# osmocom/osmo-trx

Measured on AMD Instinct MI355X. Metric: Mbursts/s detect+demod (156.25 sym, 4 SPS), higher is better.
Workload: dtype f32

## Files before the change

### osmo_trx_amd/csrc/trx_kernel_nb.hip

```cpp
#include "trx_k4_common.h"
#include "trx_nb_asm.inc"

#define NB_D_LEN    160
#define NB_CZ_LEN   (TRX_CZ_PAD + TRX_CORR_NARROW + TRX_CZ_PAD)
#define NB_SLICE    (K4_XS + NB_D_LEN + NB_CZ_LEN)
#define NB_COMP_ROWS (TRX_DELAY_FILTS + 1)
#define NB_AMP_FLOATS (8 * 8)
#define NB_TABLES_FLOATS (TRX_SINCV_LDS + 16 * WAVE + NB_COMP_ROWS * 36 + 16 + 8 * 8 + 5 * WAVE + 5 * WAVE + 2 * 8 * 16 + NB_AMP_FLOATS)
#define NB_TABLES_BYTES (NB_TABLES_FLOATS * 4)
#define NB_WPB 16
#define NB_POOL_RING 64
#define NB_POOL_UNSET (-1)
#define NB_POOL_END (-2)
#define NB_NO_BURST 0xffffffffu
#define NB_LDS_TAIL (16 + 4 * NB_POOL_RING)
#define NB_LDS_BYTES (NB_TABLES_BYTES + NB_WPB * NB_SLICE * 8 + NB_LDS_TAIL)
#define NB_MAX_TOA 32



typedef float v3f __attribute__((ext_vector_type(3)));
typedef int v4i __attribute__((ext_vector_type(4)));
typedef int v2i __attribute__((ext_vector_type(2)));
typedef __attribute__((address_space(3))) v2f lds_v2f;

template <typename T>
__device__ __forceinline__ unsigned lds_addr(const T *p)
{
	return (unsigned)(uintptr_t)(const __attribute__((address_space(3))) T *)p;
}

__device__ __forceinline__ int nb_lane_id()
{
	int lane;
	asm volatile("v_mbcnt_lo_u32_b32 %0, -1, 0\n\tv_mbcnt_hi_u32_b32 %0, -1, %0" : "=v"(lane));
	return lane;
}

__global__ void __launch_bounds__(NB_WPB * WAVE)
nb_pull4_kernel(const uint32_t *__restrict__ iq, const trxhip_burst_params *__restrict__ params,
		trxhip_burst_result *__restrict__ results, float *__restrict__ soft, const trx_tables *__restrict__ tab,
		unsigned n_bursts, float thresh, float full_scale, unsigned *__restrict__ pool_ctr, unsigned *__restrict__ redo,
		float gk5, float gk6, float gk7, float gk8)
{
	static_assert(NB_TABLES_BYTES % 16 == 0 && (NB_SLICE * 8) % 16 == 0 && (K4_XS * 8) % 16 == 0 && (NB_D_LEN * 8) % 16 == 0, "16-byte LDS accesses");
	static_assert(NB_LDS_BYTES <= 160 * 1024, "LDS");
	static_assert(NB_ASM_GDEC_OFF == (TRX_SINCV_LDS + 16 * WAVE + NB_COMP_ROWS * 36) * 4, "tools/gen_nb_asm.py: LDS offset of the decimator taps");
	static_assert(NB_ASM_DEC_MAX_NACT == 15 + NB_ASM_CORR_MAX_LEN, "tools/gen_nb_asm.py: DEC and CORR change form at the same window (one test)");
	static_assert(NB_ASM_LSEQ_OFF == (NB_TABLES_FLOATS - NB_AMP_FLOATS - 2 * 8 * 16) * 4, "tools/gen_nb_asm.py: LDS offset of the training-sequence taps");
	static_assert(NB_ASM_AW_PD == (PH_M0 + 52) * 8 && NB_ASM_AW_D == K4_XS * 8 && NB_ASM_AW_CZ == (K4_XS + NB_D_LEN + TRX_CZ_PAD) * 8,
		      "tools/gen_nb_asm.py: offsets of P, D[] and cz[] inside a wave's slice");
	constexpr int NLD = 10;
	extern __shared__ __attribute__((aligned(16))) char smem[];
	const int lane0 = threadIdx.x & (WAVE - 1);
	const int wave = uni((int)(threadIdx.x >> 6));

	float *const sincv = reinterpret_cast<float *>(smem);
	float *const wa4f = sincv + TRX_SINCV_LDS;
	const float4 *const wa4 = reinterpret_cast<const float4 *>(wa4f);
	float *const comp = wa4f + 16 * WAVE;
	float *const gdec = comp + NB_COMP_ROWS * 36;
	float *const lhdr = gdec + 16;
	int *const pkcl = reinterpret_cast<int *>(lhdr + 8 * 8);
	int *const lcn = pkcl + 5 * WAVE;
	c32 *const lseq = reinterpret_cast<c32 *>(lcn + 5 * WAVE);
	float *const lamp = reinterpret_cast<float *>(lseq + 8 * 16);
	c32 *const wbase = reinterpret_cast<c32 *>(smem + NB_TABLES_BYTES) + (size_t)wave * NB_SLICE;
	int *const wg_next = reinterpret_cast<int *>(reinterpret_cast<c32 *>(smem + NB_TABLES_BYTES) + (size_t)NB_WPB * NB_SLICE);
	int *const pool_g = wg_next + 4;
	c32 *const P = wbase;
	c32 *const D = wbase + K4_XS;
	c32 *const cz = D + NB_D_LEN + TRX_CZ_PAD;

	static_assert(4 * TRX_SINCP_STRIDE <= TRX_SINCV_LDS, "the row pairs fit the LUT's LDS space");
	for (int i = threadIdx.x; i < TRX_SINCV_LDS; i += blockDim.x) {
		const int src = trx_sincp_src(i);
		sincv[i] = (src >= 0) ? tab->sincv[src] : 0.0f;
	}
	for (int i = threadIdx.x; i < 16 * WAVE; i += blockDim.x) {
		const int l = i & (WAVE - 1), u = i >> 6;
		const PeakConst pcl = peak_const(l);
		const int q = (u < 8) ? pcl.loA + 512 * (7 - u) : pcl.hiA + 512 * (u - 8);
		wa4f[((u >> 2) * WAVE + l) * 4 + (u & 3)] = (q < TRX_SINCV_LEN) ? tab->sincv[q] : 0.0f;
	}
	for (int i = threadIdx.x; i < NB_COMP_ROWS * 36; i += blockDim.x) {
		const int f = i / 36, j = i % 36;
		comp[i] = (j >= TRX_FUSED_SH) ? tab->comp_filt[f][j - TRX_FUSED_SH] : 0.0f;
	}
	if (threadIdx.x < 16)
		gdec[threadIdx.x] = tab->dec_taps[threadIdx.x];
	if (threadIdx.x < 128)
		lseq[threadIdx.x] = make_float2(tab->seq[TRX_SEQ_TSC0 + (threadIdx.x >> 4)].taps[threadIdx.x & 15].re,
						tab->seq[TRX_SEQ_TSC0 + (threadIdx.x >> 4)].taps[threadIdx.x & 15].im);
	if (threadIdx.x < 64)
		lhdr[threadIdx.x] = reinterpret_cast<const float *>(&tab->seq[TRX_SEQ_TSC0 + (threadIdx.x >> 3)].gain)[threadIdx.x & 7];
	if (threadIdx.x < NB_AMP_FLOATS) {
		const trx_c32 gi = tab->seq[TRX_SEQ_TSC0 + (threadIdx.x >> 3)].gain_inv;
		lamp[threadIdx.x] = trx_amp_lane_coef(gi.re, gi.im, (int)(threadIdx.x & 7));
	}
	if (threadIdx.x < WAVE) {
		const PeakConst pc0 = peak_const(threadIdx.x);
		pkcl[0 * WAVE + threadIdx.x] = pc0.flA;
		pkcl[1 * WAVE + threadIdx.x] = pc0.loA;
		pkcl[2 * WAVE + threadIdx.x] = pc0.hiA;
		pkcl[3 * WAVE + threadIdx.x] = pc0.offB;
		pkcl[4 * WAVE + threadIdx.x] = pc0.ratio_off;
		lcn[2 * threadIdx.x + 0] = pc0.ratio_off * 8;
		lcn[2 * threadIdx.x + 1] = (pc0.flA - 8) * 8;
		lcn[2 * (WAVE + threadIdx.x) + 0] = pc0.offB;
		const int l = threadIdx.x, e = (l - 52) / 3, t = (l - 52) % 3;
		const bool sp = l >= 52;
		lcn[2 * (WAVE + l) + 1] = 8 * (sp ? (t == 0 ? e : t == 1 ? e + 3 : e - 3) : 4 + 3 * (l < 49 ? l : 49));
		lcn[4 * WAVE + l] = sp ? (e + (t == 2 ? 4 : 0)) * K4_NTP * 4 : -1;
	}
	for (int i = lane0; i < NB_SLICE; i += WAVE)
		wbase[i] = make_float2(0.0f, 0.0f);
	if (threadIdx.x == 0) {
		wg_next[0] = NB_WPB;
		wg_next[1] = 0;
	}
	if (threadIdx.x < NB_POOL_RING)
		pool_g[threadIdx.x] = NB_POOL_UNSET;
	__syncthreads();

	const float thr2 = thresh * thresh;
	float gkv = lane0 == 5 ? gk5 : lane0 == 6 ? gk6 : lane0 == 7 ? gk7 : gk8;
	asm volatile("" : "+v"(gkv));
	const float gc0 = thr2 * 1.0001e-5f;
	int t5pk = 0;
	bool t5_ok = true;
	for (int t = 0; t < 8; t++) {
		const int v = (int)(lhdr[8 * t + 5] * 512.0f);
		t5_ok = t5_ok && v >= -8 && v <= 7 && (float)v == lhdr[8 * t + 5] * 512.0f;
		t5pk |= (v & 15) << (4 * t);
	}
	t5pk = uni(t5pk);
	const unsigned toa_lim = (unsigned)uni(t5_ok ? (int)((NB_MAX_TOA + 1u) << 16) : 0);
	const unsigned long long e8_addr = reinterpret_cast<unsigned long long>(&tab->edge8[0][0][0]);
	const unsigned n_wg = gridDim.x;
	const unsigned n_groups = (n_bursts + 15u) >> 4;
	const bool pooled = pool_ctr != nullptr;
	const unsigned n_static_groups = pooled ? ((n_groups - (n_groups >> 3)) / n_wg) * n_wg : n_groups;
	const unsigned n_pool_groups = n_groups - n_static_groups;
	const unsigned gq = n_static_groups / n_wg, gr = n_static_groups % n_wg;
	const unsigned my_groups = gq + (blockIdx.x < gr ? 1u : 0u);
	const unsigned base16 = (blockIdx.x * gq + (blockIdx.x < gr ? blockIdx.x : gr)) << 4;
	unsigned items = my_groups << 4;
	if (base16 + items > n_bursts)
		items = (base16 < n_bursts) ? n_bursts - base16 : 0u;
	auto burst_of = [&](unsigned jj) -> unsigned {
		if (__builtin_expect(jj < items, 1))
			return base16 + jj;
		if (!pooled)
			return NB_NO_BURST;
		const unsigned k = (jj - items) >> 4;
		volatile int *slot = pool_g + (k & (NB_POOL_RING - 1));
		int g;
		while ((g = *slot) == NB_POOL_UNSET)
			__builtin_amdgcn_s_sleep(2);
		g = uni(g);
		if (g < 0)
			return NB_NO_BURST;
// ... 304 lines not shown
				int clip;
				asm("s_cmp_lg_u64 %1, 0\n\ts_cselect_b32 %0, 1, 0" : "=s"(clip) : "s"(__ballot(amax > TRX_CLIP_THRESH)) : "scc");

				const int len = 16 + (int)max_toa;
				__builtin_assume(len >= 16 && len <= 16 + NB_MAX_TOA);
				float v;
				const int lag0 = (len <= NB_ASM_CORR_MAX_LEN) ? NB_ASM_CORR_LANE0 : 0;
				asm volatile(NB_ASM_DECCORR
					     : [nrm] "=&v"(v)
					     : [aw] "v"(a_w), [zero] "v"(0), [len] "s"(len), [tsc] "s"(tsc)
					     : NB_ASM_CLOBBERS);
				{
					DIAG_MARK(3);
					int m_bits, es_bits, bidx;
					v2i kra, kbc;
					int ktp;
					asm volatile(NB_ASM_AMAX("v_lshlrev_b32_e32 v90, 1, %[l4]", "ds_read_b64 %[kra], v90 offset:%c[lc]",
								 "ds_read_b64 %[kbc], v90 offset:%c[lc]+512", "ds_read_b32 %[ktp], %[l4] offset:%c[lc]+1024",
								 "s_nop 0", "s_nop 0", "s_nop 0", "s_nop 0")
						     "s_sub_u32 %[bidx], %[bidx], %[lag0]\n\t"
						     "s_waitcnt lgkmcnt(0)"
						     : [m] "=&s"(m_bits), [es] "=&s"(es_bits), [bidx] "=&s"(bidx), [kra] "=&v"(kra), [kbc] "=&v"(kbc), [ktp] "=&v"(ktp)
						     : [nrm] "v"(v), [ep] "v"(epart), [l4] "v"(a_l4), [lag0] "s"(lag0),
						       [lc] "n"((TRX_SINCV_LDS + 16 * WAVE + NB_COMP_ROWS * 36 + 16 + 64 + 5 * WAVE) * 4)
						     : NB_ASM_CLOBBERS);
					DIAG_MARK(4);
					int st, e512;
					float km;
					asm volatile(NB_ASM_DETA
						     : [st] "=&" NB_ASM_ST(st), [e] "=&s"(e512), [km] "=&v"(km)
						     : [bidx] "s"(bidx), [len] "s"(len), [czb] "s"(lds_addr(cz)), [m] "s"(m_bits), [kr] "v"(kra.x), [ka] "v"(kra.y), [l16] "v"(a_l16),
						       [gkv] "v"(gkv), [c0] "v"(gc0)
						     : NB_ASM_CLOBBERS_ST);
					DIAG_MARK(5);
					int toa512 = 0, xr_bits = 0, xi_bits = 0;
					if (__builtin_expect(st == 1, 1)) {
						asm volatile(NB_ASM_DETB
							     : [st] "=&" NB_ASM_ST(st), [toa] "=&s"(toa512), [xr] "=&s"(xr_bits), [xi] "=&s"(xi_bits)
							     : [e] "s"(e512), [kb] "v"(kbc.x), [czb] "s"(lds_addr(cz)), [km] "v"(km)
							     : NB_ASM_CLOBBERS_ST);
						DIAG_MARK(6);
					}
					if (__builtin_expect(st != 1, 0)) {
						int stc = st;
						asm volatile("" : "+s"(stc));
						if (stc == 3) {
							const int lane = nb_lane_id();
							if (lane == 0)
								atomicAdd(&g_trx_fast_stats[0], 1ull);
							PeakConst pkc;
							pkc.flA = pkcl[0 * WAVE + lane]; pkc.loA = pkcl[1 * WAVE + lane]; pkc.hiA = pkcl[2 * WAVE + lane];
							pkc.offB = pkcl[3 * WAVE + lane]; pkc.ratio_off = pkcl[4 * WAVE + lane];
							c32 xcorr;
							peak_detect_spec<true>(cz, bidx, sincv, pkc, lane, &toa512, &xcorr, wa4);
							toa512 = uni(toa512);
							xr_bits = uni(__float_as_int(xcorr.x));
							xi_bits = uni(__float_as_int(xcorr.y));
							st = 1;
						} else if (stc == 2) {
							if (nb_lane_id() == 0) atomicAdd(&g_trx_fast_stats[2], 1ull);
							mark_left(b);
							keep = 0;
						} else {
							const float energy = __int_as_float(es_bits) * 0.0125f;
							const float rssi = rssi_db(full_scale, energy);
							const uint32_t flags = ((uint32_t)clip << 8) | (1u << 16);
							int word = clip ? -TRXHIP_SIGERR_CLIP : 0;
							word = put_lane<1>(word, 0.0f);
							word = put_lane<2>(word, 0.0f);
							word = put_lane<3>(word, 0.0f);
							word = put_lane<4>(word, 0.0f);
							word = put_lane<5>(word, energy);
							word = put_lane<6>(word, rssi);
							word = write_lane<7>(word, (int)flags);
							recw = word;
							o = (v3f){ 0.0f, 0.0f, 0.0f };
							pend_rm = 0xff;
						}
					}
					if (__builtin_expect(st == 1, 1)) {
						int ok, s_bits;
						float d0, d1, d2;
						const int t5 = (t5pk << (28 - 4 * tsc)) >> 28;
						asm volatile("s_setprio 0");
						asm volatile(NB_ASM_TAIL
							     : [ok] "=&s"(ok), [ssum] "=&s"(s_bits), [d0] "=&v"(d0), [d1] "=&v"(d1), [d2] "=&v"(d2)
							     : [toa] "s"(toa512), [xr] "s"(xr_bits), [xi] "s"(xi_bits), [t5] "s"(t5), [ampb] "s"(lds_addr(lamp) + 32u * (unsigned)tsc),
							       [e8lo] "s"((unsigned)e8_addr), [e8hi] "s"((unsigned)(e8_addr >> 32)), [l16] "v"(a_l16), [l4] "v"(a_l4),
							       [aw] "v"(a_w), [pb] "s"(lds_addr(P)), [cb] "s"(lds_addr(comp) + 4u * (K4_U0 + TRX_FUSED_SH)), [db] "s"(lds_addr(D)),
							       [kic] "v"(kbc.y), [ktp] "v"(ktp)
							     : NB_ASM_CLOBBERS);
						DIAG_MARK(10);
						asm volatile("s_setprio 2");
						o.x = d0;
						o.y = d1;
						o.z = d2;
						queue_record(xr_bits, xi_bits, es_bits, toa512 - t5 - 10 * 512, s_bits,
							     (int)((uint32_t)tsc | ((uint32_t)clip << 8) | (37u << 24)), b);
						if (__builtin_expect(!ok, 0)) {
							const int lane = nb_lane_id();
							if (lane == 0) atomicAdd(&g_trx_fast_stats[3], 1ull);
							const float *const h = lhdr + 8 * tsc;
							const float xr = __int_as_float(xr_bits), xi = __int_as_float(xi_bits);
							const float a0 = xr * h[2], a1 = xr * h[3], a2 = xi * h[3], a3 = xi * h[2];
							const c32 ampv = make_float2(unif(a0 - a2), unif(a1 + a3));
							if (!demod_general(t5 + 10 * 512 - toa512, ampv, lane)) {
								q_n--;
// ... 32 lines not shown
```

### osmo_trx_amd/csrc/trx_nb_asm.inc

```
#define NB_ASM_GDEC_OFF 29968
#define NB_ASM_LSEQ_OFF 32848
#define NB_ASM_DEC_MAX_NACT 60
#define NB_ASM_CORR_LANE0 19
#define NB_ASM_CORR_MAX_LEN 45
#define NB_ASM_AW_PD 512
#define NB_ASM_AW_D 5760
#define NB_ASM_AW_CZ 7136
#define NB_ASM_ST "{s98}"
#define NB_ASM_CLOBBERS "v64", "v65", "v66", "v67", "v68", "v69", "v70", "v71", "v72", "v73", "v74", "v75", "v76", "v77", "v78", "v79", "v80", "v81", "v82", "v83", "v84", "v85", "v86", "v87", "v88", "v89", "v90", "v91", "v92", "v93", "v94", "v95", "v96", "v97", "v98", "v99", "v100", "v101", "v102", "v103", "v104", "v105", "v106", "v107", "v108", "v109", "v110", "v111", "v112", "v113", "v114", "v115", "v116", "v117", "v118", "v119", "v120", "v121", "v122", "v123", "v124", "v125", "v126", "v127", "s87", "s88", "s89", "s90", "s91", "s92", "s93", "s94", "s95", "s96", "s97", "s98", "s99", "vcc", "scc", "memory"
#define NB_ASM_CLOBBERS_ST "v64", "v65", "v66", "v67", "v68", "v69", "v70", "v71", "v72", "v73", "v74", "v75", "v76", "v77", "v78", "v79", "v80", "v81", "v82", "v83", "v84", "v85", "v86", "v87", "v88", "v89", "v90", "v91", "v92", "v93", "v94", "v95", "v96", "v97", "v98", "v99", "v100", "v101", "v102", "v103", "v104", "v105", "v106", "v107", "v108", "v109", "v110", "v111", "v112", "v113", "v114", "v115", "v116", "v117", "v118", "v119", "v120", "v121", "v122", "v123", "v124", "v125", "v126", "v127", "s87", "s88", "s89", "s90", "s91", "s92", "s93", "s94", "s95", "s96", "s97", "s99", "vcc", "scc", "memory"
#define NB_ASM_DECCORR \
	"s_add_u32 s92, %[len], 15\n\t" \
	"s_cmp_gt_u32 %[len], 45\n\t" \
	"s_cbranch_scc1 .Lnbc_dc_wide\n\t" \
	"s_sub_u32 s88, 60, s92\n\t" \
	"s_lshr_b64 exec, -1, s88\n\t" \
	"ds_read_b128 v[120:123], %[zero] offset:29968\n\t" \
	"ds_read_b128 v[124:127], %[zero] offset:29984\n\t" \
	"ds_read_b64 v[98:99], %[aw] offset:1952\n\t" \
	"ds_read_b64 v[100:101], %[aw] offset:3392\n\t" \
	"ds_read_b64 v[102:103], %[aw] offset:4832\n\t" \
	"ds_read_b64 v[96:97], %[aw] offset:512\n\t" \
	"s_waitcnt lgkmcnt(3)\n\t" \
	"v_pk_mul_f32 v[64:65], v[98:99], v[120:121] op_sel:[0,0] op_sel_hi:[1,0]\n\t" \
// ... 1180 lines not shown
	"ds_read_b64 v[102:103], v66 offset:56\n\t" \
	"v_mov_b32_e32 v74, %[m]\n\t" \
	"s_add_u32 s91, %[bidx], -1\n\t" \
	"s_sub_u32 s92, %[len], %[bidx]\n\t" \
	"s_min_u32 s91, s91, 4\n\t" \
	"v_mul_f32_e32 %[km], 0x36c9539c, v74\n\t" \
	"s_add_u32 s92, s92, -2\n\t" \
	"s_waitcnt lgkmcnt(11)\n\t" \
	"s_bfm_b64 exec, 8, 0\n\t" \
	"v_pk_mul_f32 v[70:71], v[70:71], v[70:71]\n\t" \
	"s_min_u32 s92, s92, 4\n\t" \
	"v_add_f32_e32 v75, v71, v70\n\t" \
	"s_add_u32 s91, s91, s92\n\t" \
	"v_readlane_b32 s92, %[gkv], s91\n\t" \
	"v_add_f32_dpp v75, v75, v75 quad_perm:[1,0,3,2] row_mask:0xf bank_mask:0xf\n\t" \
	"s_nop 1\n\t" \
	"v_add_f32_dpp v75, v75, v75 quad_perm:[2,3,0,1] row_mask:0xf bank_mask:0xf\n\t" \
	"s_nop 1\n\t" \
	"v_add_f32_dpp v75, v75, v75 row_half_mirror row_mask:0xf bank_mask:0xf\n\t" \
	"v_mul_f32_e32 v112, s92, v75\n\t" \
	"v_mul_f32_e32 v113, 0x3f7fff37, v112\n\t" \
	"v_fmamk_f32 v114, v112, 0x3f8000c9, %[c0]\n\t" \
	"v_cmp_gt_f32_e32 vcc, v74, v114\n\t" \
	"s_cbranch_vccz .Lnbc_da_gate\n\t" \
	"s_mov_b64 exec, -1\n\t" \
	"ds_read_b128 v[104:107], %[l16] offset:18560\n\t" \
	"ds_read_b128 v[108:111], %[l16] offset:19584\n\t" \
	"ds_read_b64 v[112:113], v66 offset:64\n\t" \
	"ds_read_b64 v[114:115], v66 offset:72\n\t" \
	"ds_read_b64 v[116:117], v66 offset:80\n\t" \
	"ds_read_b64 v[118:119], v66 offset:88\n\t" \
	"ds_read_b64 v[120:121], v66 offset:96\n\t" \
	"ds_read_b64 v[122:123], v66 offset:104\n\t" \
	"ds_read_b64 v[124:125], v66 offset:112\n\t" \
	"ds_read_b64 v[126:127], v66 offset:120\n\t" \
	"s_waitcnt lgkmcnt(10)\n\t" \
	"v_pk_mul_f32 v[84:85], v[88:89], v[76:77] op_sel:[0,0] op_sel_hi:[1,0]\n\t" \
	"v_pk_mul_f32 v[86:87], v[90:91], v[76:77] op_sel:[0,1] op_sel_hi:[1,1]\n\t" \
	"v_pk_fma_f32 v[84:85], v[92:93], v[78:79], v[84:85] op_sel:[0,0,0] op_sel_hi:[1,0,1]\n\t" \
	"v_pk_fma_f32 v[86:87], v[94:95], v[78:79], v[86:87] op_sel:[0,1,0] op_sel_hi:[1,1,1]\n\t" \
	"v_pk_fma_f32 v[84:85], v[96:97], v[80:81], v[84:85] op_sel:[0,0,0] op_sel_hi:[1,0,1]\n\t" \
	"v_pk_fma_f32 v[86:87], v[98:99], v[80:81], v[86:87] op_sel:[0,1,0] op_sel_hi:[1,1,1]\n\t" \
	"v_pk_fma_f32 v[84:85], v[100:101], v[82:83], v[84:85] op_sel:[0,0,0] op_sel_hi:[1,0,1]\n\t" \
	"v_pk_fma_f32 v[86:87], v[102:103], v[82:83], v[86:87] op_sel:[0,1,0] op_sel_hi:[1,1,1]\n\t" \
	"s_waitcnt lgkmcnt(0)\n\t" \
	"v_pk_fma_f32 v[84:85], v[112:113], v[104:105], v[84:85] op_sel:[0,0,0] op_sel_hi:[1,0,1]\n\t" \
	"v_pk_fma_f32 v[86:87], v[114:115], v[104:105], v[86:87] op_sel:[0,1,0] op_sel_hi:[1,1,1]\n\t" \
	"v_pk_fma_f32 v[84:85], v[116:117], v[106:107], v[84:85] op_sel:[0,0,0] op_sel_hi:[1,0,1]\n\t" \
	"v_pk_fma_f32 v[86:87], v[118:119], v[106:107], v[86:87] op_sel:[0,1,0] op_sel_hi:[1,1,1]\n\t" \
	"v_pk_fma_f32 v[84:85], v[120:121], v[108:109], v[84:85] op_sel:[0,0,0] op_sel_hi:[1,0,1]\n\t" \
	"v_pk_fma_f32 v[86:87], v[122:123], v[108:109], v[86:87] op_sel:[0,1,0] op_sel_hi:[1,1,1]\n\t" \
	"v_pk_fma_f32 v[84:85], v[124:125], v[110:111], v[84:85] op_sel:[0,0,0] op_sel_hi:[1,0,1]\n\t" \
	"v_pk_fma_f32 v[86:87], v[126:127], v[110:111], v[86:87] op_sel:[0,1,0] op_sel_hi:[1,1,1]\n\t" \
	"s_nop 0\n\t" \
	"v_pk_add_f32 v[84:85], v[84:85], v[86:87]\n\t" \
	"s_nop 0\n\t" \
	"v_pk_mul_f32 v[84:85], v[84:85], v[84:85]\n\t" \
	"s_nop 0\n\t" \
	"v_add_f32_e32 v88, v85, v84\n\t" \
	"v_fmamk_f32 v89, v88, 0x36c9539c, %[km]\n\t" \
	"v_sub_f32_e32 v90, v88, v89\n\t" \
	"v_add_f32_e32 v91, v88, v89\n\t" \
	"s_lshl_b32 s94, %[bidx], 9\n\t" \
	"v_mov_b32_dpp v90, v90 quad_perm:[1,0,3,2] row_mask:0xf bank_mask:0xf\n\t" \
	"v_cmp_lt_f32_e64 s[88:89], v91, v90\n\t" \
	"s_mov_b32 s98, 1\n\t" \
	"s_lshr_b64 s[90:91], s[88:89], 1\n\t" \
	"s_or_b64 s[90:91], s[90:91], s[88:89]\n\t" \
	"s_mov_b32 s96, 0x55555555\n\t" \
	"s_mov_b32 s97, 0x15555555\n\t" \
	"s_and_b64 s[92:93], s[90:91], s[96:97]\n\t" \
	"s_cmp_eq_u64 s[92:93], s[96:97]\n\t" \
	"s_cbranch_scc0 .Lnbc_da_careful\n\t" \
	"s_mov_b32 s95, 0\n\t" \
	"s_lshl1_add_u32 s96, s95, 0\n\t" \
	"s_bitcmp1_b64 s[88:89], s96\n\t" \
	"s_addc_u32 s95, s95, s95\n\t" \
	"s_lshl1_add_u32 s96, s95, 2\n\t" \
	"s_bitcmp1_b64 s[88:89], s96\n\t" \
	"s_addc_u32 s95, s95, s95\n\t" \
	"s_lshl1_add_u32 s96, s95, 6\n\t" \
	"s_bitcmp1_b64 s[88:89], s96\n\t" \
	"s_addc_u32 s95, s95, s95\n\t" \
	"s_lshl1_add_u32 s96, s95, 14\n\t" \
	"s_bitcmp1_b64 s[88:89], s96\n\t" \
	"s_addc_u32 s95, s95, s95\n\t" \
	"s_lshl1_add_u32 s96, s95, 30\n\t" \
	"s_bitcmp1_b64 s[88:89], s96\n\t" \
	"s_addc_u32 s95, s95, s95\n\t" \
	".Lnb_da_walked:\n\t" \
	"s_lshl_b32 s95, s95, 5\n\t" \
	"s_add_u32 s94, s94, s95\n\t" \
	"s_add_u32 %[e], s94, -1008\n\t" \
	".Lnb_da_end:\n\t"
#define NB_ASM_DETB \
	"v_add_u32_e32 v68, %[e], %[kb]\n\t" \
	"s_add_u32 s88, %[czb], -56\n\t" \
	"s_mov_b32 exec_lo, 0x3fffffff\n\t" \
	"s_mov_b32 exec_hi, 0xffff\n\t" \
	"v_ashrrev_i32_e32 v69, 9, v68\n\t" \
	"v_and_b32_e32 v70, 0x1ff, v68\n\t" \
	"v_lshl_add_u32 v69, v69, 3, s88\n\t" \
	"v_bfe_u32 v71, v70, 4, 5\n\t" \
	"v_sub_u32_e32 v72, 0x200, v70\n\t" \
	"v_xor_b32_e32 v71, v71, v70\n\t" \
	"v_bfe_u32 v73, v72, 4, 5\n\t" \
	"v_lshlrev_b32_e32 v71, 3, v71\n\t" \
	"v_xor_b32_e32 v72, v73, v72\n\t" \
	"v_lshlrev_b32_e32 v72, 3, v72\n\t" \
	"ds_read_b64 v[80:81], v69 offset:0\n\t" \
	"ds_read_b64 v[96:97], v71 offset:12312\n\t" \
	"ds_read_b64 v[82:83], v69 offset:8\n\t" \
	"ds_read_b64 v[84:85], v69 offset:16\n\t" \
	"ds_read_b64 v[98:99], v71 offset:8208\n\t" \
	"ds_read_b64 v[86:87], v69 offset:24\n\t" \
	"ds_read_b64 v[88:89], v69 offset:32\n\t" \
	"ds_read_b64 v[100:101], v71 offset:4104\n\t" \
	"ds_read_b64 v[90:91], v69 offset:40\n\t" \
	"ds_read_b64 v[92:93], v69 offset:48\n\t" \
	"ds_read_b64 v[102:103], v71 offset:0\n\t" \
	"ds_read_b64 v[94:95], v69 offset:56\n\t" \
	"s_waitcnt lgkmcnt(9)\n\t" \
	"v_pk_mul_f32 v[64:65], v[80:81], v[96:97] op_sel:[0,1] op_sel_hi:[1,1]\n\t" \
	"v_pk_mul_f32 v[66:67], v[82:83], v[96:97] op_sel:[0,0] op_sel_hi:[1,0]\n\t" \
	"ds_read_b64 v[104:105], v69 offset:64\n\t" \
	"ds_read_b64 v[120:121], v72 offset:0\n\t" \
	"ds_read_b64 v[106:107], v69 offset:72\n\t" \
	"s_waitcnt lgkmcnt(9)\n\t" \
	"v_pk_fma_f32 v[64:65], v[84:85], v[98:99], v[64:65] op_sel:[0,1,0] op_sel_hi:[1,1,1]\n\t" \
	"v_pk_fma_f32 v[66:67], v[86:87], v[98:99], v[66:67] op_sel:[0,0,0] op_sel_hi:[1,0,1]\n\t" \
	"ds_read_b64 v[108:109], v69 offset:80\n\t" \
	"ds_read_b64 v[122:123], v72 offset:4104\n\t" \
	"ds_read_b64 v[110:111], v69 offset:88\n\t" \
	"s_waitcnt lgkmcnt(9)\n\t" \
	"v_pk_fma_f32 v[64:65], v[88:89], v[100:101], v[64:65] op_sel:[0,1,0] op_sel_hi:[1,1,1]\n\t" \
	"v_pk_fma_f32 v[66:67], v[90:91], v[100:101], v[66:67] op_sel:[0,0,0] op_sel_hi:[1,0,1]\n\t" \
	"ds_read_b64 v[112:113], v69 offset:96\n\t" \
	"ds_read_b64 v[124:125], v72 offset:8208\n\t" \
	"ds_read_b64 v[114:115], v69 offset:104\n\t" \
	"s_waitcnt lgkmcnt(9)\n\t" \
	"v_pk_fma_f32 v[64:65], v[92:93], v[102:103], v[64:65] op_sel:[0,1,0] op_sel_hi:[1,1,1]\n\t" \
	"v_pk_fma_f32 v[66:67], v[94:95], v[102:103], v[66:67] op_sel:[0,0,0] op_sel_hi:[1,0,1]\n\t" \
	"ds_read_b64 v[116:117], v69 offset:112\n\t" \
	"ds_read_b64 v[126:127], v72 offset:12312\n\t" \
	"ds_read_b64 v[118:119], v69 offset:120\n\t" \
	"s_waitcnt lgkmcnt(9)\n\t" \
	"v_pk_fma_f32 v[64:65], v[104:105], v[120:121], v[64:65] op_sel:[0,0,0] op_sel_hi:[1,0,1]\n\t" \
	"v_pk_fma_f32 v[66:67], v[106:107], v[120:121], v[66:67] op_sel:[0,1,0] op_sel_hi:[1,1,1]\n\t" \
	"s_waitcnt lgkmcnt(6)\n\t" \
	"v_pk_fma_f32 v[64:65], v[108:109], v[122:123], v[64:65] op_sel:[0,0,0] op_sel_hi:[1,0,1]\n\t" \
	"v_pk_fma_f32 v[66:67], v[110:111], v[122:123], v[66:67] op_sel:[0,1,0] op_sel_hi:[1,1,1]\n\t" \
	"s_waitcnt lgkmcnt(3)\n\t" \
	"v_pk_fma_f32 v[64:65], v[112:113], v[124:125], v[64:65] op_sel:[0,0,0] op_sel_hi:[1,0,1]\n\t" \
	"v_pk_fma_f32 v[66:67], v[114:115], v[124:125], v[66:67] op_sel:[0,1,0] op_sel_hi:[1,1,1]\n\t" \
	"s_waitcnt lgkmcnt(0)\n\t" \
	"v_pk_fma_f32 v[64:65], v[116:117], v[126:127], v[64:65] op_sel:[0,0,0] op_sel_hi:[1,0,1]\n\t" \
	"v_pk_fma_f32 v[66:67], v[118:119], v[126:127], v[66:67] op_sel:[0,1,0] op_sel_hi:[1,1,1]\n\t" \
	"s_mov_b64 exec, -1\n\t" \
	"v_pk_add_f32 v[74:75], v[64:65], v[66:67]\n\t" \
	"s_add_u32 s92, %[e], 497\n\t" \
	"v_pk_mul_f32 v[76:77], v[74:75], v[74:75]\n\t" \
	"s_mov_b32 s98, 1\n\t" \
	"v_add_f32_e32 v78, v77, v76\n\t" \
	"v_fmamk_f32 v79, v78, 0x36c9539c, %[km]\n\t" \
	"v_sub_f32_e32 v96, v78, v79\n\t" \
	"v_add_f32_e32 v97, v78, v79\n\t" \
	"s_nop 0\n\t" \
	"v_mov_b32_dpp v96, v96 quad_perm:[1,0,3,2] row_mask:0xf bank_mask:0xf\n\t" \
	"v_cmp_lt_f32_e64 s[88:89], v97, v96\n\t" \
	"s_lshr_b32 s90, s88, 1\n\t" \
	"s_or_b32 s90, s90, s88\n\t" \
	"s_and_b32 s91, s90, 0x15555555\n\t" \
	"s_cmp_eq_u32 s91, 0x15555555\n\t" \
	"s_cbranch_scc0 .Lnbc_db_careful\n\t" \
	"s_mov_b32 s94, 0\n\t" \
	"s_lshl1_add_u32 s95, s94, 0\n\t" \
	"s_bitcmp1_b32 s88, s95\n\t" \
	"s_addc_u32 s94, s94, s94\n\t" \
	"s_lshl1_add_u32 s95, s94, 2\n\t" \
	"s_bitcmp1_b32 s88, s95\n\t" \
	"s_addc_u32 s94, s94, s94\n\t" \
	"s_lshl1_add_u32 s95, s94, 6\n\t" \
	"s_bitcmp1_b32 s88, s95\n\t" \
	"s_addc_u32 s94, s94, s94\n\t" \
	"s_lshl1_add_u32 s95, s94, 14\n\t" \
	"s_bitcmp1_b32 s88, s95\n\t" \
	"s_addc_u32 s94, s94, s94\n\t" \
	".Lnb_db_walked:\n\t" \
	"s_add_u32 s93, s94, 32\n\t" \
	"s_lshl1_add_u32 %[toa], s94, s92\n\t" \
	"v_readlane_b32 %[xr], v74, s93\n\t" \
	"v_readlane_b32 %[xi], v75, s93\n\t" \
	".Lnb_db_end:\n\t"
#define NB_ASM_TAIL \
	"v_and_or_b32 v65, %[l4], 12, %[ampb]\n\t" \
	"ds_read2_b32 v[70:71], v65 offset1:4\n\t" \
	"s_sub_u32 s88, %[t5], %[toa]\n\t" \
	"s_add_u32 s87, s88, 5120\n\t" \
	"s_mov_b32 %[ok], 0\n\t" \
	"s_and_b32 s91, s87, 127\n\t" \
	"s_lshr_b32 s99, s91, 1\n\t" \
	"s_cmp_ge_u32 s91, 2\n\t" \
	"s_cselect_b32 s99, s99, 64\n\t" \
	"s_mul_i32 s93, s99, 768\n\t" \
	"s_add_u32 s94, %[e8lo], s93\n\t" \
	"s_addc_u32 s95, %[e8hi], 0\n\t" \
	"s_abs_i32 s96, %[toa]\n\t" \
	"s_add_u32 s96, s96, 256\n\t" \
	"global_load_dwordx4 v[120:123], %[l16], s[94:95]\n\t" \
	"s_lshr_b32 s96, s96, 9\n\t" \
	"s_sub_u32 s97, 0, s96\n\t" \
	"s_cmp_lt_i32 %[toa], 0\n\t" \
	"s_cselect_b32 s96, s97, s96\n\t" \
	"s_lshl_b32 s96, s96, 3\n\t" \
	"v_add_u32_e32 v64, s96, %[aw]\n\t" \
	"s_bfm_b64 exec, 16, 0\n\t" \
	"ds_read_b64 v[66:67], v64 offset:5760\n\t" \
	"s_mov_b64 exec, -1\n\t" \
	"s_bfm_b64 exec, 16, 0\n\t" \
	"s_waitcnt lgkmcnt(0)\n\t" \
	"v_pk_mul_f32 v[66:67], v[66:67], v[66:67]\n\t" \
	"s_ashr_i32 s88, s87, 7\n\t" \
	"v_add_f32_e32 v81, v67, v66\n\t" \
	"s_sub_u32 s91, -18, s88\n\t" \
	"s_and_b32 s92, s91, 3\n\t" \
	"v_add_f32_dpp v81, v81, v81 quad_perm:[1,0,3,2] row_mask:0xf bank_mask:0xf\n\t" \
	"s_ashr_i32 s93, s91, 2\n\t" \
	"s_mul_i32 s94, s92, 180\n\t" \
	"v_add_f32_dpp v81, v81, v81 quad_perm:[2,3,0,1] row_mask:0xf bank_mask:0xf\n\t" \
	"s_add_u32 s94, s94, s93\n\t" \
	"s_lshl3_add_u32 s94, s94, %[pb]\n\t" \
	"v_add_f32_dpp v81, v81, v81 row_half_mirror row_mask:0xf bank_mask:0xf\n\t" \
	"s_mul_i32 s95, s99, 144\n\t" \
	"s_add_u32 s95, s95, %[cb]\n\t" \
	"v_add_f32_dpp v81, v81, v81 row_mirror row_mask:0xf bank_mask:0xf\n\t" \
	"s_sub_u32 s96, 0, s88\n\t" \
	"v_readlane_b32 %[ssum], v81, 0\n\t" \
	"s_mov_b64 exec, -1\n\t" \
	"s_cmp_gt_u32 s96, 36\n\t" \
	"s_cbranch_scc1 .Lnbc_tl_wait\n\t" \
	"s_mov_b32 %[ok], 1\n\t" \
	"v_add_u32_e32 v112, s94, %[kic]\n\t" \
	"s_cmp_gt_u32 s92, 2\n\t" \
// ... 250 lines not shown
	"ds_read_b128 v[104:107], v117 offset:64\n\t" \
	"ds_read_b64 v[88:89], v112 offset:144\n\t" \
	"ds_read_b64 v[90:91], v113 offset:144\n\t" \
	"ds_read_b64 v[92:93], v114 offset:144\n\t" \
	"ds_read_b64 v[94:95], v115 offset:144\n\t" \
	"s_waitcnt lgkmcnt(5)\n\t" \
	"v_pk_fma_f32 %[a0], v[96:97], v[108:109], %[a0] op_sel:[0,0,0] op_sel_hi:[1,0,1]\n\t" \
	"v_pk_fma_f32 %[a1], v[72:73], v[108:109], %[a1] op_sel:[0,0,0] op_sel_hi:[1,0,1]\n\t" \
	"v_pk_fma_f32 %[a2], v[80:81], v[108:109], %[a2] op_sel:[0,0,0] op_sel_hi:[1,0,1]\n\t" \
	"v_pk_fma_f32 %[a0], v[98:99], v[108:109], %[a0] op_sel:[0,1,0] op_sel_hi:[1,1,1]\n\t" \
	"v_pk_fma_f32 %[a1], v[74:75], v[108:109], %[a1] op_sel:[0,1,0] op_sel_hi:[1,1,1]\n\t" \
	"v_pk_fma_f32 %[a2], v[82:83], v[108:109], %[a2] op_sel:[0,1,0] op_sel_hi:[1,1,1]\n\t" \
	"v_pk_fma_f32 %[a0], v[100:101], v[110:111], %[a0] op_sel:[0,0,0] op_sel_hi:[1,0,1]\n\t" \
	"v_pk_fma_f32 %[a1], v[76:77], v[110:111], %[a1] op_sel:[0,0,0] op_sel_hi:[1,0,1]\n\t" \
	"v_pk_fma_f32 %[a2], v[84:85], v[110:111], %[a2] op_sel:[0,0,0] op_sel_hi:[1,0,1]\n\t" \
	"v_pk_fma_f32 %[a0], v[102:103], v[110:111], %[a0] op_sel:[0,1,0] op_sel_hi:[1,1,1]\n\t" \
	"v_pk_fma_f32 %[a1], v[78:79], v[110:111], %[a1] op_sel:[0,1,0] op_sel_hi:[1,1,1]\n\t" \
	"v_pk_fma_f32 %[a2], v[86:87], v[110:111], %[a2] op_sel:[0,1,0] op_sel_hi:[1,1,1]\n\t" \
	"ds_read_b128 v[108:111], v117 offset:80\n\t" \
	"ds_read_b64 v[96:97], v112 offset:152\n\t" \
	"ds_read_b64 v[98:99], v113 offset:152\n\t" \
	"ds_read_b64 v[100:101], v114 offset:152\n\t" \
	"ds_read_b64 v[102:103], v115 offset:152\n\t" \
	"s_waitcnt lgkmcnt(5)\n\t" \
	"v_pk_fma_f32 %[a0], v[72:73], v[104:105], %[a0] op_sel:[0,0,0] op_sel_hi:[1,0,1]\n\t" \
	"v_pk_fma_f32 %[a1], v[80:81], v[104:105], %[a1] op_sel:[0,0,0] op_sel_hi:[1,0,1]\n\t" \
	"v_pk_fma_f32 %[a2], v[88:89], v[104:105], %[a2] op_sel:[0,0,0] op_sel_hi:[1,0,1]\n\t" \
	"v_pk_fma_f32 %[a0], v[74:75], v[104:105], %[a0] op_sel:[0,1,0] op_sel_hi:[1,1,1]\n\t" \
	"v_pk_fma_f32 %[a1], v[82:83], v[104:105], %[a1] op_sel:[0,1,0] op_sel_hi:[1,1,1]\n\t" \
	"v_pk_fma_f32 %[a2], v[90:91], v[104:105], %[a2] op_sel:[0,1,0] op_sel_hi:[1,1,1]\n\t" \
	"v_pk_fma_f32 %[a0], v[76:77], v[106:107], %[a0] op_sel:[0,0,0] op_sel_hi:[1,0,1]\n\t" \
	"v_pk_fma_f32 %[a1], v[84:85], v[106:107], %[a1] op_sel:[0,0,0] op_sel_hi:[1,0,1]\n\t" \
	"v_pk_fma_f32 %[a2], v[92:93], v[106:107], %[a2] op_sel:[0,0,0] op_sel_hi:[1,0,1]\n\t" \
	"v_pk_fma_f32 %[a0], v[78:79], v[106:107], %[a0] op_sel:[0,1,0] op_sel_hi:[1,1,1]\n\t" \
	"v_pk_fma_f32 %[a1], v[86:87], v[106:107], %[a1] op_sel:[0,1,0] op_sel_hi:[1,1,1]\n\t" \
	"v_pk_fma_f32 %[a2], v[94:95], v[106:107], %[a2] op_sel:[0,1,0] op_sel_hi:[1,1,1]\n\t" \
	"s_waitcnt lgkmcnt(0)\n\t" \
	"v_pk_fma_f32 %[a0], v[80:81], v[108:109], %[a0] op_sel:[0,0,0] op_sel_hi:[1,0,1]\n\t" \
	"v_pk_fma_f32 %[a1], v[88:89], v[108:109], %[a1] op_sel:[0,0,0] op_sel_hi:[1,0,1]\n\t" \
	"v_pk_fma_f32 %[a2], v[96:97], v[108:109], %[a2] op_sel:[0,0,0] op_sel_hi:[1,0,1]\n\t" \
	"v_pk_fma_f32 %[a0], v[82:83], v[108:109], %[a0] op_sel:[0,1,0] op_sel_hi:[1,1,1]\n\t" \
	"v_pk_fma_f32 %[a1], v[90:91], v[108:109], %[a1] op_sel:[0,1,0] op_sel_hi:[1,1,1]\n\t" \
	"v_pk_fma_f32 %[a2], v[98:99], v[108:109], %[a2] op_sel:[0,1,0] op_sel_hi:[1,1,1]\n\t" \
	"v_pk_fma_f32 %[a0], v[84:85], v[110:111], %[a0] op_sel:[0,0,0] op_sel_hi:[1,0,1]\n\t" \
	"v_pk_fma_f32 %[a1], v[92:93], v[110:111], %[a1] op_sel:[0,0,0] op_sel_hi:[1,0,1]\n\t" \
	"v_pk_fma_f32 %[a2], v[100:101], v[110:111], %[a2] op_sel:[0,0,0] op_sel_hi:[1,0,1]\n\t" \
	"v_pk_fma_f32 %[a0], v[86:87], v[110:111], %[a0] op_sel:[0,1,0] op_sel_hi:[1,1,1]\n\t" \
	"v_pk_fma_f32 %[a1], v[94:95], v[110:111], %[a1] op_sel:[0,1,0] op_sel_hi:[1,1,1]\n\t" \
	"v_pk_fma_f32 %[a2], v[102:103], v[110:111], %[a2] op_sel:[0,1,0] op_sel_hi:[1,1,1]\n\t" \
	"s_mov_b64 exec, -1\n\t"
#define NB_ASM_COLD \
	"s_branch .Lnbc_end\n\t" \
	".Lnbc_da_careful:\n\t" \
	"s_mov_b32 s95, 0\n\t" \
	"s_lshl1_add_u32 s96, s95, 0\n\t" \
	"s_bitcmp0_b64 s[90:91], s96\n\t" \
	"s_cbranch_scc1 .Lnbc_da_unsure\n\t" \
	"s_bitcmp1_b64 s[88:89], s96\n\t" \
	"s_addc_u32 s95, s95, s95\n\t" \
	"s_lshl1_add_u32 s96, s95, 2\n\t" \
	"s_bitcmp0_b64 s[90:91], s96\n\t" \
	"s_cbranch_scc1 .Lnbc_da_unsure\n\t" \
	"s_bitcmp1_b64 s[88:89], s96\n\t" \
	"s_addc_u32 s95, s95, s95\n\t" \
	"s_lshl1_add_u32 s96, s95, 6\n\t" \
	"s_bitcmp0_b64 s[90:91], s96\n\t" \
	"s_cbranch_scc1 .Lnbc_da_unsure\n\t" \
	"s_bitcmp1_b64 s[88:89], s96\n\t" \
	"s_addc_u32 s95, s95, s95\n\t" \
	"s_lshl1_add_u32 s96, s95, 14\n\t" \
	"s_bitcmp0_b64 s[90:91], s96\n\t" \
	"s_cbranch_scc1 .Lnbc_da_unsure\n\t" \
	"s_bitcmp1_b64 s[88:89], s96\n\t" \
	"s_addc_u32 s95, s95, s95\n\t" \
	"s_lshl1_add_u32 s96, s95, 30\n\t" \
	"s_bitcmp0_b64 s[90:91], s96\n\t" \
	"s_cbranch_scc1 .Lnbc_da_unsure\n\t" \
	"s_bitcmp1_b64 s[88:89], s96\n\t" \
	"s_addc_u32 s95, s95, s95\n\t" \
	"s_branch .Lnb_da_walked\n\t" \
	".Lnbc_da_unsure:\n\t" \
	"s_mov_b32 s98, 3\n\t" \
	"s_branch .Lnb_da_end\n\t" \
	".Lnbc_da_gate:\n\t" \
	"v_cmp_lt_f32_e32 vcc, v74, v113\n\t" \
	"s_cmp_eq_u64 vcc, 0\n\t" \
	"s_cselect_b32 s98, 2, 0\n\t" \
	"s_mov_b64 exec, -1\n\t" \
	"s_waitcnt lgkmcnt(0)\n\t" \
	"s_branch .Lnb_da_end\n\t" \
	".Lnbc_db_careful:\n\t" \
	"s_mov_b32 s94, 0\n\t" \
	"s_lshl1_add_u32 s95, s94, 0\n\t" \
	"s_bitcmp0_b32 s90, s95\n\t" \
	"s_cbranch_scc1 .Lnbc_db_unsure\n\t" \
	"s_bitcmp1_b32 s88, s95\n\t" \
	"s_addc_u32 s94, s94, s94\n\t" \
	"s_lshl1_add_u32 s95, s94, 2\n\t" \
	"s_bitcmp0_b32 s90, s95\n\t" \
	"s_cbranch_scc1 .Lnbc_db_unsure\n\t" \
	"s_bitcmp1_b32 s88, s95\n\t" \
	"s_addc_u32 s94, s94, s94\n\t" \
	"s_lshl1_add_u32 s95, s94, 6\n\t" \
	"s_bitcmp0_b32 s90, s95\n\t" \
	"s_cbranch_scc1 .Lnbc_db_unsure\n\t" \
	"s_bitcmp1_b32 s88, s95\n\t" \
	"s_addc_u32 s94, s94, s94\n\t" \
	"s_lshl1_add_u32 s95, s94, 14\n\t" \
	"s_bitcmp0_b32 s90, s95\n\t" \
	"s_cbranch_scc1 .Lnbc_db_unsure\n\t" \
	"s_bitcmp1_b32 s88, s95\n\t" \
	"s_addc_u32 s94, s94, s94\n\t" \
	"s_branch .Lnb_db_walked\n\t" \
	".Lnbc_db_unsure:\n\t" \
	"s_mov_b32 s98, 3\n\t" \
	"s_branch .Lnb_db_end\n\t" \
	".Lnbc_tl_wait:\n\t" \
	"s_waitcnt vmcnt(0)\n\t" \
	"s_branch .Lnb_tl_end\n\t" \
	".Lnbc_end:\n\t"
#define NB_ASM_AMAX(FILL0, FILL1, FILL2, FILL3, FILL4, FILL5, FILL6, FILL7) \
	"v_mov_b32_e32 v88, %[nrm]\n\t" \
	"v_mov_b32_dpp v89, %[ep] quad_perm:[0,0,0,0] row_mask:0xf bank_mask:0xf\n\t" \
	FILL0 "\n\t" \
	"v_max_f32_dpp v88, v88, v88 quad_perm:[1,0,3,2] row_mask:0xf bank_mask:0xf\n\t" \
	"v_add_f32_dpp v89, v89, v89 row_half_mirror row_mask:0xf bank_mask:0xf\n\t" \
	FILL1 "\n\t" \
	"v_max_f32_dpp v88, v88, v88 quad_perm:[2,3,0,1] row_mask:0xf bank_mask:0xf\n\t" \
	"v_add_f32_dpp v89, v89, v89 row_mirror row_mask:0xf bank_mask:0xf\n\t" \
	FILL2 "\n\t" \
	"v_max_f32_dpp v88, v88, v88 row_half_mirror row_mask:0xf bank_mask:0xf\n\t" \
	"v_add_f32_dpp v89, v89, v89 row_bcast:15 row_mask:0xa bank_mask:0xf\n\t" \
	FILL3 "\n\t" \
	"v_max_f32_dpp v88, v88, v88 row_mirror row_mask:0xf bank_mask:0xf\n\t" \
	"v_add_f32_dpp v89, v89, v89 row_bcast:31 row_mask:0xc bank_mask:0xf\n\t" \
	FILL4 "\n\t" \
	"v_max_f32_dpp v88, v88, v88 row_bcast:15 row_mask:0xa bank_mask:0xf\n\t" \
	FILL5 "\n\t" \
	"v_readlane_b32 %[es], v89, 63\n\t" \
	"v_max_f32_dpp v88, v88, v88 row_bcast:31 row_mask:0xc bank_mask:0xf\n\t" \
	FILL6 "\n\t" \
	FILL7 "\n\t" \
	"v_readlane_b32 %[m], v88, 63\n\t" \
	"s_nop 1\n\t" \
	"v_cmp_eq_f32_e32 vcc, %[m], %[nrm]\n\t" \
	"s_ff1_i32_b64 %[bidx], vcc\n\t"
```

Measured before the change: 1191.

## Reorder peak-search lanes so tree walk becomes a find-first-zero scan

Permutes how the per-lane peak-search candidates are assigned to lanes. The binary tree of pairwise comparisons is laid out in order by level rather than in heap order, and the wavefront walk that descends it is replaced by an xor against an alternating pattern, a find-first-zero, and a mask check. This removes a serial chain of five (or four) dependent scalar bit tests per detection. The table setup, the fallback search's lane index, and the cold careful paths are all remapped to match the new lane permutation. The risk is correctness if any table indexed by lane was left unpermuted.

```diff
diff --git a/osmo_trx_amd/csrc/trx_kernel_nb.hip b/osmo_trx_amd/csrc/trx_kernel_nb.hip
--- a/osmo_trx_amd/csrc/trx_kernel_nb.hip
+++ b/osmo_trx_amd/csrc/trx_kernel_nb.hip
@@ -35,6 +35,26 @@
 	int lane;
 	asm volatile("v_mbcnt_lo_u32_b32 %0, -1, 0\n\tv_mbcnt_hi_u32_b32 %0, -1, %0" : "=v"(lane));
 	return lane;
+}
+
+template <int LEVELS>
+__device__ __forceinline__ int nb_walk_src(int l)
+{
+	const int r = l >> 1;
+	if (r >= (1 << LEVELS) - 1)
+		return l;
+	const int t = __ffs(r + 1) - 1;
+	const int k = LEVELS - 1 - t, i = (r + 1) >> (t + 1);
+	return 2 * ((1 << k) - 1 + i) + (l & 1);
+}
+template <int LEVELS>
+__device__ __forceinline__ int nb_walk_dst(int l)
+{
+	const int n = l >> 1;
+	if (n >= (1 << LEVELS) - 1)
+		return l;
+	const int k = 31 - __clz(n + 1), i = n + 1 - (1 << k);
+	return 2 * (((2 * i + 1) << (LEVELS - 1 - k)) - 1) + (l & 1);
 }
 
 __global__ void __launch_bounds__(NB_WPB * WAVE)
@@ -79,7 +99,7 @@
 	}
 	for (int i = threadIdx.x; i < 16 * WAVE; i += blockDim.x) {
 		const int l = i & (WAVE - 1), u = i >> 6;
-		const PeakConst pcl = peak_const(l);
+		const PeakConst pcl = peak_const(nb_walk_src<5>(l));
 		const int q = (u < 8) ? pcl.loA + 512 * (7 - u) : pcl.hiA + 512 * (u - 8);
 		wa4f[((u >> 2) * WAVE + l) * 4 + (u & 3)] = (q < TRX_SINCV_LEN) ? tab->sincv[q] : 0.0f;
 	}
@@ -106,8 +126,8 @@
 		pkcl[3 * WAVE + threadIdx.x] = pc0.offB;
 		pkcl[4 * WAVE + threadIdx.x] = pc0.ratio_off;
 		lcn[2 * threadIdx.x + 0] = pc0.ratio_off * 8;
-		lcn[2 * threadIdx.x + 1] = (pc0.flA - 8) * 8;
-		lcn[2 * (WAVE + threadIdx.x) + 0] = pc0.offB;
+		lcn[2 * threadIdx.x + 1] = (peak_const(nb_walk_src<5>((int)threadIdx.x)).flA - 8) * 8;
+		lcn[2 * (WAVE + threadIdx.x) + 0] = peak_const(nb_walk_src<4>((int)threadIdx.x)).offB;
 		const int l = threadIdx.x, e = (l - 52) / 3, t = (l - 52) % 3;
 		const bool sp = l >= 52;
 		lcn[2 * (WAVE + l) + 1] = 8 * (sp ? (t == 0 ? e : t == 1 ? e + 3 : e - 3) : 4 + 3 * (l < 49 ? l : 49));
@@ -518,7 +538,7 @@
 							pkc.flA = pkcl[0 * WAVE + lane]; pkc.loA = pkcl[1 * WAVE + lane]; pkc.hiA = pkcl[2 * WAVE + lane];
 							pkc.offB = pkcl[3 * WAVE + lane]; pkc.ratio_off = pkcl[4 * WAVE + lane];
 							c32 xcorr;
-							peak_detect_spec<true>(cz, bidx, sincv, pkc, lane, &toa512, &xcorr, wa4);
+							peak_detect_spec<true>(cz, bidx, sincv, pkc, nb_walk_dst<5>(lane), &toa512, &xcorr, wa4);
 							toa512 = uni(toa512);
 							xr_bits = uni(__float_as_int(xcorr.x));
 							xi_bits = uni(__float_as_int(xcorr.y));
diff --git a/osmo_trx_amd/csrc/trx_nb_asm.inc b/osmo_trx_amd/csrc/trx_nb_asm.inc
--- a/osmo_trx_amd/csrc/trx_nb_asm.inc
+++ b/osmo_trx_amd/csrc/trx_nb_asm.inc
@@ -1256,11 +1256,11 @@
 	"v_pk_fma_f32 v[86:87], v[122:123], v[108:109], v[86:87] op_sel:[0,1,0] op_sel_hi:[1,1,1]\n\t" \
 	"v_pk_fma_f32 v[84:85], v[124:125], v[110:111], v[84:85] op_sel:[0,0,0] op_sel_hi:[1,0,1]\n\t" \
 	"v_pk_fma_f32 v[86:87], v[126:127], v[110:111], v[86:87] op_sel:[0,1,0] op_sel_hi:[1,1,1]\n\t" \
-	"s_nop 0\n\t" \
+	"s_mov_b32 s96, 0xaaaaaaaa\n\t" \
 	"v_pk_add_f32 v[84:85], v[84:85], v[86:87]\n\t" \
-	"s_nop 0\n\t" \
+	"s_mov_b32 s97, 0x2aaaaaaa\n\t" \
 	"v_pk_mul_f32 v[84:85], v[84:85], v[84:85]\n\t" \
-	"s_nop 0\n\t" \
+	"s_mov_b32 s98, 1\n\t" \
 	"v_add_f32_e32 v88, v85, v84\n\t" \
 	"v_fmamk_f32 v89, v88, 0x36c9539c, %[km]\n\t" \
 	"v_sub_f32_e32 v90, v88, v89\n\t" \
@@ -1268,33 +1268,14 @@
 	"s_lshl_b32 s94, %[bidx], 9\n\t" \
 	"v_mov_b32_dpp v90, v90 quad_perm:[1,0,3,2] row_mask:0xf bank_mask:0xf\n\t" \
 	"v_cmp_lt_f32_e64 s[88:89], v91, v90\n\t" \
-	"s_mov_b32 s98, 1\n\t" \
-	"s_lshr_b64 s[90:91], s[88:89], 1\n\t" \
-	"s_or_b64 s[90:91], s[90:91], s[88:89]\n\t" \
-	"s_mov_b32 s96, 0x55555555\n\t" \
-	"s_mov_b32 s97, 0x15555555\n\t" \
-	"s_and_b64 s[92:93], s[90:91], s[96:97]\n\t" \
-	"s_cmp_eq_u64 s[92:93], s[96:97]\n\t" \
+	"s_bfe_u64 s[90:91], s[88:89], 0x3e0000\n\t" \
+	"s_xor_b64 s[90:91], s[90:91], s[96:97]\n\t" \
+	"s_ff0_i32_b64 s95, s[90:91]\n\t" \
+	"s_bfm_b64 s[92:93], s95, 0\n\t" \
+	"s_cmp_eq_u64 s[92:93], s[90:91]\n\t" \
 	"s_cbranch_scc0 .Lnbc_da_careful\n\t" \
-	"s_mov_b32 s95, 0\n\t" \
-	"s_lshl1_add_u32 s96, s95, 0\n\t" \
-	"s_bitcmp1_b64 s[88:89], s96\n\t" \
-	"s_addc_u32 s95, s95, s95\n\t" \
-	"s_lshl1_add_u32 s96, s95, 2\n\t" \
-	"s_bitcmp1_b64 s[88:89], s96\n\t" \
-	"s_addc_u32 s95, s95, s95\n\t" \
-	"s_lshl1_add_u32 s96, s95, 6\n\t" \
-	"s_bitcmp1_b64 s[88:89], s96\n\t" \
-	"s_addc_u32 s95, s95, s95\n\t" \
-	"s_lshl1_add_u32 s96, s95, 14\n\t" \
-	"s_bitcmp1_b64 s[88:89], s96\n\t" \
-	"s_addc_u32 s95, s95, s95\n\t" \
-	"s_lshl1_add_u32 s96, s95, 30\n\t" \
-	"s_bitcmp1_b64 s[88:89], s96\n\t" \
-	"s_addc_u32 s95, s95, s95\n\t" \
 	".Lnb_da_walked:\n\t" \
-	"s_lshl_b32 s95, s95, 5\n\t" \
-	"s_add_u32 s94, s94, s95\n\t" \
+	"s_lshl4_add_u32 s94, s95, s94\n\t" \
 	"s_add_u32 %[e], s94, -1008\n\t" \
 	".Lnb_da_end:\n\t"
 #define NB_ASM_DETB \
@@ -1372,27 +1353,16 @@
 	"s_nop 0\n\t" \
 	"v_mov_b32_dpp v96, v96 quad_perm:[1,0,3,2] row_mask:0xf bank_mask:0xf\n\t" \
 	"v_cmp_lt_f32_e64 s[88:89], v97, v96\n\t" \
-	"s_lshr_b32 s90, s88, 1\n\t" \
-	"s_or_b32 s90, s90, s88\n\t" \
-	"s_and_b32 s91, s90, 0x15555555\n\t" \
-	"s_cmp_eq_u32 s91, 0x15555555\n\t" \
+	"s_and_b32 s90, s88, 0x3fffffff\n\t" \
+	"s_xor_b32 s90, s90, 0x2aaaaaaa\n\t" \
+	"s_ff0_i32_b32 s94, s90\n\t" \
+	"s_bfm_b32 s91, s94, 0\n\t" \
+	"s_cmp_eq_u32 s91, s90\n\t" \
 	"s_cbranch_scc0 .Lnbc_db_careful\n\t" \
-	"s_mov_b32 s94, 0\n\t" \
-	"s_lshl1_add_u32 s95, s94, 0\n\t" \
-	"s_bitcmp1_b32 s88, s95\n\t" \
-	"s_addc_u32 s94, s94, s94\n\t" \
-	"s_lshl1_add_u32 s95, s94, 2\n\t" \
-	"s_bitcmp1_b32 s88, s95\n\t" \
-	"s_addc_u32 s94, s94, s94\n\t" \
-	"s_lshl1_add_u32 s95, s94, 6\n\t" \
-	"s_bitcmp1_b32 s88, s95\n\t" \
-	"s_addc_u32 s94, s94, s94\n\t" \
-	"s_lshl1_add_u32 s95, s94, 14\n\t" \
-	"s_bitcmp1_b32 s88, s95\n\t" \
-	"s_addc_u32 s94, s94, s94\n\t" \
 	".Lnb_db_walked:\n\t" \
-	"s_add_u32 s93, s94, 32\n\t" \
-	"s_lshl1_add_u32 %[toa], s94, s92\n\t" \
+	"s_lshr_b32 s93, s94, 1\n\t" \
+	"s_add_u32 %[toa], s94, s92\n\t" \
+	"s_add_u32 s93, s93, 32\n\t" \
 	"v_readlane_b32 %[xr], v74, s93\n\t" \
 	"v_readlane_b32 %[xi], v75, s93\n\t" \
 	".Lnb_db_end:\n\t"
@@ -1749,32 +1719,40 @@
 #define NB_ASM_COLD \
 	"s_branch .Lnbc_end\n\t" \
 	".Lnbc_da_careful:\n\t" \
+	"s_lshr_b64 s[90:91], s[88:89], 1\n\t" \
+	"s_or_b64 s[90:91], s[90:91], s[88:89]\n\t" \
 	"s_mov_b32 s95, 0\n\t" \
-	"s_lshl1_add_u32 s96, s95, 0\n\t" \
+	"s_lshl_b32 s96, s95, 6\n\t" \
+	"s_add_u32 s96, s96, 30\n\t" \
 	"s_bitcmp0_b64 s[90:91], s96\n\t" \
 	"s_cbranch_scc1 .Lnbc_da_unsure\n\t" \
 	"s_bitcmp1_b64 s[88:89], s96\n\t" \
 	"s_addc_u32 s95, s95, s95\n\t" \
-	"s_lshl1_add_u32 s96, s95, 2\n\t" \
+	"s_lshl_b32 s96, s95, 5\n\t" \
+	"s_add_u32 s96, s96, 14\n\t" \
 	"s_bitcmp0_b64 s[90:91], s96\n\t" \
 	"s_cbranch_scc1 .Lnbc_da_unsure\n\t" \
 	"s_bitcmp1_b64 s[88:89], s96\n\t" \
 	"s_addc_u32 s95, s95, s95\n\t" \
-	"s_lshl1_add_u32 s96, s95, 6\n\t" \
+	"s_lshl_b32 s96, s95, 4\n\t" \
+	"s_add_u32 s96, s96, 6\n\t" \
 	"s_bitcmp0_b64 s[90:91], s96\n\t" \
 	"s_cbranch_scc1 .Lnbc_da_unsure\n\t" \
 	"s_bitcmp1_b64 s[88:89], s96\n\t" \
 	"s_addc_u32 s95, s95, s95\n\t" \
-	"s_lshl1_add_u32 s96, s95, 14\n\t" \
+	"s_lshl_b32 s96, s95, 3\n\t" \
+	"s_add_u32 s96, s96, 2\n\t" \
 	"s_bitcmp0_b64 s[90:91], s96\n\t" \
 	"s_cbranch_scc1 .Lnbc_da_unsure\n\t" \
 	"s_bitcmp1_b64 s[88:89], s96\n\t" \
 	"s_addc_u32 s95, s95, s95\n\t" \
-	"s_lshl1_add_u32 s96, s95, 30\n\t" \
+	"s_lshl_b32 s96, s95, 2\n\t" \
+	"s_add_u32 s96, s96, 0\n\t" \
 	"s_bitcmp0_b64 s[90:91], s96\n\t" \
 	"s_cbranch_scc1 .Lnbc_da_unsure\n\t" \
 	"s_bitcmp1_b64 s[88:89], s96\n\t" \
 	"s_addc_u32 s95, s95, s95\n\t" \
+	"s_lshl_b32 s95, s95, 1\n\t" \
 	"s_branch .Lnb_da_walked\n\t" \
 	".Lnbc_da_unsure:\n\t" \
 	"s_mov_b32 s98, 3\n\t" \
@@ -1787,27 +1765,34 @@
 	"s_waitcnt lgkmcnt(0)\n\t" \
 	"s_branch .Lnb_da_end\n\t" \
 	".Lnbc_db_careful:\n\t" \
+	"s_lshr_b32 s90, s88, 1\n\t" \
+	"s_or_b32 s90, s90, s88\n\t" \
 	"s_mov_b32 s94, 0\n\t" \
-	"s_lshl1_add_u32 s95, s94, 0\n\t" \
+	"s_lshl_b32 s95, s94, 5\n\t" \
+	"s_add_u32 s95, s95, 14\n\t" \
 	"s_bitcmp0_b32 s90, s95\n\t" \
 	"s_cbranch_scc1 .Lnbc_db_unsure\n\t" \
 	"s_bitcmp1_b32 s88, s95\n\t" \
 	"s_addc_u32 s94, s94, s94\n\t" \
-	"s_lshl1_add_u32 s95, s94, 2\n\t" \
+	"s_lshl_b32 s95, s94, 4\n\t" \
+	"s_add_u32 s95, s95, 6\n\t" \
 	"s_bitcmp0_b32 s90, s95\n\t" \
 	"s_cbranch_scc1 .Lnbc_db_unsure\n\t" \
 	"s_bitcmp1_b32 s88, s95\n\t" \
 	"s_addc_u32 s94, s94, s94\n\t" \
-	"s_lshl1_add_u32 s95, s94, 6\n\t" \
+	"s_lshl_b32 s95, s94, 3\n\t" \
+	"s_add_u32 s95, s95, 2\n\t" \
 	"s_bitcmp0_b32 s90, s95\n\t" \
 	"s_cbranch_scc1 .Lnbc_db_unsure\n\t" \
 	"s_bitcmp1_b32 s88, s95\n\t" \
 	"s_addc_u32 s94, s94, s94\n\t" \
-	"s_lshl1_add_u32 s95, s94, 14\n\t" \
+	"s_lshl_b32 s95, s94, 2\n\t" \
+	"s_add_u32 s95, s95, 0\n\t" \
 	"s_bitcmp0_b32 s90, s95\n\t" \
 	"s_cbranch_scc1 .Lnbc_db_unsure\n\t" \
 	"s_bitcmp1_b32 s88, s95\n\t" \
 	"s_addc_u32 s94, s94, s94\n\t" \
+	"s_lshl_b32 s94, s94, 1\n\t" \
 	"s_branch .Lnb_db_walked\n\t" \
 	".Lnbc_db_unsure:\n\t" \
 	"s_mov_b32 s98, 3\n\t" \
```

Result: faster. 1207, median of 6 (+1.3%).
